# brown-palm/goal-force

Measured on AMD Instinct MI355X. Metric: frames_per_sec (81-frame video / (50-step denoise loop + VAE decode), Wan2.2-I2V-A14B 832x480x81f), higher is better.
Workload: dtype bf16

## Files before the change

goal_force_amd/csrc/gf_cross_fold.hip:

```cpp
#include "gf_common.h"

namespace {

constexpr int CF_HD = 128;
constexpr int CF_MAXK = 64;
constexpr int CF_THREADS = 256;
constexpr int CF_QB = 128;

__device__ __forceinline__ void cf_mfma32(f32x16& acc, const bf16x8& a, const bf16x8& b) {
    acc = __builtin_amdgcn_mfma_f32_32x32x16_bf16(a, b, acc, 0, 0, 0);
}

__global__ __launch_bounds__(CF_THREADS) void cross_probs_kernel(const u16* __restrict__ q, const u16* __restrict__ k, u16* __restrict__ pout,
                                                                 int q_len, int n_keys, int n_pad, int heads, long q_stride, long k_stride,
                                                                 long p_stride, float c, float last_key_bias) {
    __shared__ __attribute__((aligned(16))) char lds[CF_MAXK * 256];
    const int tid = threadIdx.x;
    const int lane = tid & 63, wave = tid >> 6;
    const int r = lane & 31, h = lane >> 5;
    const int head = blockIdx.y;
    const int q0 = blockIdx.x * CF_QB + wave * 32;
    const int halves = n_keys > 32 ? 2 : 1;

#pragma unroll
    for (int i = 0; i < (CF_MAXK * 16) / CF_THREADS; ++i) {
        const int idx = tid + CF_THREADS * i;
        const int row = idx >> 4, ch = idx & 15;
        u16x8 v8 = {0, 0, 0, 0, 0, 0, 0, 0};
        if (row < n_keys) v8 = *reinterpret_cast<const u16x8*>(k + (long)row * k_stride + head * CF_HD + ch * 8);
        const int sk = ((row & 3) << 2) | ((row >> 2) & 3);
        *(u16x8*)(lds + row * 256 + ((ch ^ sk) << 4)) = v8;
    }

    bf16x8 qf[8];
    {
        const int qr = min(q0 + r, q_len - 1);
        const u16* qp = q + (long)qr * q_stride + head * CF_HD + 8 * h;
#pragma unroll
        for (int kd = 0; kd < 8; ++kd) qf[kd] = *reinterpret_cast<const bf16x8*>(qp + 16 * kd);
    }
    __syncthreads();

    f32x16 sc[2];
#pragma unroll
    for (int e = 0; e < 16; ++e) {
        sc[0][e] = 0.f;
        sc[1][e] = 0.f;
    }
    const int sK = ((r & 3) << 2) | ((r >> 2) & 3);
#pragma unroll
    for (int kd = 0; kd < 8; ++kd) {
        const int off = 256 * r + 16 * ((2 * kd + h) ^ sK);
        cf_mfma32(sc[0], *(const bf16x8*)(lds + off), qf[kd]);
        if (halves == 2) cf_mfma32(sc[1], *(const bf16x8*)(lds + off + 32 * 256), qf[kd]);
    }

#pragma unroll
    for (int e = 0; e < 16; ++e) {
        const int key = 4 * h + (e & 3) + 8 * (e >> 2);
        if (key >= n_keys) sc[0][e] = -INFINITY;
        if (key + 32 >= n_keys) sc[1][e] = -INFINITY;
        if (key == n_keys - 1) sc[0][e] += last_key_bias;
        if (key + 32 == n_keys - 1) sc[1][e] += last_key_bias;
    }
    float mx = sc[0][0];
#pragma unroll
    for (int e = 1; e < 16; ++e) mx = fmaxf(mx, sc[0][e]);
#pragma unroll
    for (int e = 0; e < 16; ++e) mx = fmaxf(mx, sc[1][e]);
    mx = fmaxf(mx, __shfl_xor(mx, 32));
    const float mc = mx * c;
    float rs = 0.f;
#pragma unroll
    for (int e = 0; e < 16; ++e) {
        sc[0][e] = __builtin_amdgcn_exp2f(__builtin_fmaf(sc[0][e], c, -mc));
        sc[1][e] = __builtin_amdgcn_exp2f(__builtin_fmaf(sc[1][e], c, -mc));
        rs += sc[0][e] + sc[1][e];
    }
    const float l_tot = rs + __shfl_xor(rs, 32);
    const float inv = 1.0f / l_tot;
    float pl = 0.f;
#pragma unroll
    for (int e = 0; e < 16; ++e) {
        const int key = 4 * h + (e & 3) + 8 * (e >> 2);
        if (key == n_keys - 1) pl = sc[0][e];
        if (key + 32 == n_keys - 1) pl = sc[1][e];
    }
    pl += __shfl_xor(pl, 32);
    const float wl = pl * inv;
    const float wl_lo = wl - bf2f(f2bf(wl));

    const int qrow = q0 + r;
    if (qrow < q_len) {
        u16* prow = pout + (long)qrow * p_stride + (long)head * n_pad;
#pragma unroll
        for (int half = 0; half < 2; ++half)
#pragma unroll
            for (int g = 0; g < 4; ++g) {
                const int key = 32 * half + 8 * g + 4 * h;
                if (key < n_pad) {
                    float w4[4];
#pragma unroll
                    for (int i = 0; i < 4; ++i) w4[i] = key + i == n_keys ? wl_lo : sc[half][4 * g + i] * inv;
                    u32x2 pk;
                    pk[0] = pack2bf(w4[0], w4[1]);
                    pk[1] = pack2bf(w4[2], w4[3]);
                    *reinterpret_cast<u32x2*>(prow + key) = pk;
                }
            }
    }
}

constexpr int CFT_ROWS = 64;
__global__ __launch_bounds__(CF_THREADS) void cross_fold_table_kernel(const u16* __restrict__ v, const u16* __restrict__ w, u16* __restrict__ u,
                                                                      int n_keys, int n_pad, int n_out, long v_stride, long w_stride,
                                                                      long u_stride) {
    __shared__ __attribute__((aligned(16))) u16 vs[CF_MAXK * CF_HD];
    const int tid = threadIdx.x;
    const int head = blockIdx.y;
    for (int idx = tid; idx < n_pad * 16; idx += CF_THREADS) {
        const int row = idx >> 4, ch = idx & 15;
        u16x8 v8 = {0, 0, 0, 0, 0, 0, 0, 0};
        if (row <= n_keys) v8 = *reinterpret_cast<const u16x8*>(v + (long)min(row, n_keys - 1) * v_stride + head * CF_HD + ch * 8);
        *reinterpret_cast<u16x8*>(vs + row * CF_HD + ch * 8) = v8;
    }
    __syncthreads();
    const int n = blockIdx.x * CFT_ROWS + (tid >> 2), jg = tid & 3;
    if (n >= n_out) return;
    const int nj = n_pad >> 2;
    float acc[CF_MAXK / 4];
#pragma unroll
    for (int i = 0; i < CF_MAXK / 4; ++i) acc[i] = 0.f;
    const u16* wr = w + (long)n * w_stride + head * CF_HD;
    for (int d0 = 0; d0 < CF_HD; d0 += 8) {
        const u16x8 w8 = *reinterpret_cast<const u16x8*>(wr + d0);
        float wf[8];
#pragma unroll
        for (int e = 0; e < 8; ++e) wf[e] = bf2f(w8[e]);
#pragma unroll
        for (int i = 0; i < CF_MAXK / 4; ++i) {
            if (i < nj) {
                const u16x8 v8 = *reinterpret_cast<const u16x8*>(vs + (jg + 4 * i) * CF_HD + d0);
#pragma unroll
                for (int e = 0; e < 8; ++e) acc[i] = __builtin_fmaf(bf2f(v8[e]), wf[e], acc[i]);
            }
        }
    }
    u16* ur = u + (long)n * u_stride + (long)head * n_pad;
#pragma unroll
    for (int i = 0; i < CF_MAXK / 4; ++i) {
        const int j = jg + 4 * i;
        if (i < nj) ur[j] = j <= n_keys ? f2bf(acc[i]) : (u16)0;
    }
}

}

extern "C" GF_API int gf_cross_probs(const void* q, const void* k, void* p, int64_t q_len, int64_t n_keys, int64_t n_pad, int64_t heads,
                                     int64_t head_dim, int64_t q_stride, int64_t k_stride, int64_t p_stride, float scale,
                                     float last_key_multiplicity, void* stream) {
    GF_CHECK_ARG(q && k && p, "gf_cross_probs: null pointer");
    if (head_dim != CF_HD) {
        gf_set_error("gf_cross_probs: head_dim=%ld unsupported (kernel is built for 128)", (long)head_dim);
        return GF_ERR_UNSUPPORTED;
    }
    GF_CHECK_ARG(q_len >= 0 && q_len < (1 << 30) && heads > 0 && heads < 65536, "gf_cross_probs: bad sizes q=%ld heads=%ld", (long)q_len,
                 (long)heads);
    GF_CHECK_ARG(n_keys >= 1 && n_pad % 16 == 0 && n_pad > n_keys && n_pad <= CF_MAXK,
                 "gf_cross_probs: 1 <= n_keys=%ld < n_pad=%ld <= 64, n_pad a multiple of 16", (long)n_keys, (long)n_pad);
    GF_CHECK_ARG(q_stride % 8 == 0 && k_stride % 8 == 0 && p_stride % 4 == 0 && q_stride >= heads * CF_HD && k_stride >= heads * CF_HD &&
                     p_stride >= heads * n_pad,
                 "gf_cross_probs: strides must cover the rows (q, k: multiples of 8; p: of 4, >= heads * n_pad)");
    GF_CHECK_ARG(gf_aligned16(q) && gf_aligned16(k) && ((uintptr_t)p & 7u) == 0, "gf_cross_probs: alignment (q, k 16 bytes, p 8 bytes)");
    GF_CHECK_ARG(scale > 0.f && last_key_multiplicity >= 1.0f, "gf_cross_probs: scale > 0, multiplicity >= 1");
    if (q_len == 0) return GF_OK;
    const float c = scale * 1.4426950408889634f;
    const float bias = last_key_multiplicity != 1.0f ? log2f(last_key_multiplicity) / c : 0.f;
    const dim3 grid((unsigned)((q_len + CF_QB - 1) / CF_QB), (unsigned)heads);
    hipLaunchKernelGGL(cross_probs_kernel, grid, dim3(CF_THREADS), 0, (hipStream_t)stream, (const u16*)q, (const u16*)k, (u16*)p,
                       (int)q_len, (int)n_keys, (int)n_pad, (int)heads, (long)q_stride, (long)k_stride, (long)p_stride, c, bias);
    GF_CHECK_LAUNCH("gf_cross_probs");
    return GF_OK;
}

extern "C" GF_API int gf_cross_fold_table(const void* v, const void* w_o, void* u, int64_t n_keys, int64_t n_pad, int64_t heads,
                                          int64_t head_dim, int64_t n_out, int64_t v_stride, int64_t w_stride, int64_t u_stride,
                                          void* stream) {
    GF_CHECK_ARG(v && w_o && u, "gf_cross_fold_table: null pointer");
    if (head_dim != CF_HD) {
        gf_set_error("gf_cross_fold_table: head_dim=%ld unsupported (kernel is built for 128)", (long)head_dim);
        return GF_ERR_UNSUPPORTED;
    }
    GF_CHECK_ARG(heads > 0 && heads < 65536 && n_out > 0 && n_out < (1 << 30), "gf_cross_fold_table: bad sizes heads=%ld N=%ld", (long)heads,
                 (long)n_out);
    GF_CHECK_ARG(n_keys >= 1 && n_pad % 16 == 0 && n_pad > n_keys && n_pad <= CF_MAXK,
                 "gf_cross_fold_table: 1 <= n_keys=%ld < n_pad=%ld <= 64, n_pad a multiple of 16", (long)n_keys, (long)n_pad);
    GF_CHECK_ARG(v_stride % 8 == 0 && w_stride % 8 == 0 && v_stride >= heads * CF_HD && w_stride >= heads * CF_HD && u_stride >= heads * n_pad,
                 "gf_cross_fold_table: strides must cover the rows (v, w_o: multiples of 8; u >= heads * n_pad)");
    GF_CHECK_ARG(gf_aligned16(v) && gf_aligned16(w_o) && ((uintptr_t)u & 1u) == 0, "gf_cross_fold_table: alignment");
    const dim3 grid((unsigned)((n_out + CFT_ROWS - 1) / CFT_ROWS), (unsigned)heads);
    hipLaunchKernelGGL(cross_fold_table_kernel, grid, dim3(CF_THREADS), 0, (hipStream_t)stream, (const u16*)v, (const u16*)w_o, (u16*)u,
                       (int)n_keys, (int)n_pad, (int)n_out, (long)v_stride, (long)w_stride, (long)u_stride);
    GF_CHECK_LAUNCH("gf_cross_fold_table");
    return GF_OK;
}
```

goal_force_amd/dit.py:

```python
from __future__ import annotations

import math
from typing import Optional, Tuple

import torch
import torch.nn as nn

from . import ops
from ._lib import GoalForceError


def precompute_freqs_cis(dim: int, end: int = 1024, theta: float = 10000.0):
    freqs = 1.0 / (theta ** (torch.arange(0, dim, 2)[: (dim // 2)].double() / dim))
    freqs = torch.outer(torch.arange(end), freqs)
    return torch.polar(torch.ones_like(freqs), freqs)


def precompute_freqs_cis_3d(dim: int, end: int = 1024, theta: float = 10000.0):
    return (precompute_freqs_cis(dim - 2 * (dim // 3), end, theta),
            precompute_freqs_cis(dim // 3, end, theta),
            precompute_freqs_cis(dim // 3, end, theta))


class RopeTable:
# ... 283 lines not shown
        x2 = _tokens2d(x)
        a = self.attend(x2, _as_rope(freqs, x.device))
        return linear(a, self.o).view(x.shape)


class CrossAttention(nn.Module):

    def __init__(self, dim: int, num_heads: int, eps: float = 1e-6, has_image_input: bool = False):
        super().__init__()
        if has_image_input:
            raise NotImplementedError("has_image_input=True (CLIP image tokens) is outside the Goal-Force path")
        self.dim, self.num_heads, self.head_dim = dim, num_heads, dim // num_heads
        self.q, self.k, self.v, self.o = (nn.Linear(dim, dim) for _ in range(4))
        self.norm_q, self.norm_k = RMSNorm(dim, eps=eps), RMSNorm(dim, eps=eps)
        self.has_image_input = False

    def context_kv(self, ctx2: torch.Tensor, fold: bool = True, pad_n: Optional[int] = None):
        m = 1
        if fold and ctx2.is_cuda and ops._OPT["fold_pad_keys"]:
            n = pad_run(ctx2) if pad_n is None else pad_n
            if ctx2.shape[0] - n >= 2 and n + 1 < ops.VT_MIN_KV:
                m = ctx2.shape[0] - n
                ctx2 = ctx2[: n + 1]
        cin = QuantizedInput(ctx2) if getattr(self.k, "_gf_w8", None) is not None else ctx2
        k, v = linear(cin, self.k), linear(cin, self.v)
        ops.rmsnorm_rope(k, self.norm_k.weight, None, None, self.head_dim, self.norm_k.eps)
        return k, v, m

    def attend(self, x2, kv):
        q = linear(x2, self.q)
        ops.rmsnorm_rope(q, self.norm_q.weight, None, None, self.head_dim, self.norm_q.eps)
        return ops.flash_attn(q, kv[0], kv[1], self.num_heads, last_key_mult=kv[2] if len(kv) > 2 else 1)

    FOLD_K_MAX = 2560

    def fold_ok(self, kv) -> bool:
        if not ops._OPT["fold_cross_o"] or torch.is_grad_enabled() or len(kv) < 3 or kv[2] == 1 or self.head_dim != 128:
            return False
        if getattr(self.o, "_gf_w8", None) is not None:
            return False
        n = kv[0].shape[0]
        k = self.num_heads * self.fold_pad(n)
        return n <= ops.CROSS_FOLD_MAX_KEYS and k <= self.FOLD_K_MAX and k % 64 == 0

    @staticmethod
    def fold_pad(n_keys: int) -> int:
        return -(-(n_keys + 1) // 16) * 16

    def fold_table(self, kv):
        return ops.cross_fold_table(kv[1], self.o.weight, self.num_heads, self.fold_pad(kv[0].shape[0]))

    def attend_probs(self, x2, kv):
        q = linear(x2, self.q)
        ops.rmsnorm_rope(q, self.norm_q.weight, None, None, self.head_dim, self.norm_q.eps)
        return ops.cross_probs(q, kv[0], self.num_heads, self.fold_pad(kv[0].shape[0]), last_key_mult=kv[2])

    def forward(self, x: torch.Tensor, y: torch.Tensor):
        x2 = _tokens2d(x)
        a = self.attend(x2, self.context_kv(_tokens2d(y)))
        return linear(a, self.o).view(x.shape)


class GateModule(nn.Module):

    def forward(self, x, gate, residual):
        if x.shape != residual.shape:
            raise GoalForceError("GateModule: x and residual must have the same shape")
        d = x.shape[-1]
        g = gate.reshape(-1, d)
        if x.dim() == 3 and g.shape[0] == x.shape[0] and x.shape[0] > 1:
            return torch.stack([ops.gate_residual(x[b], g[b].contiguous(), residual[b]) for b in range(x.shape[0])])
        if g.shape[0] != 1:
            raise GoalForceError("GateModule: gate must be [B or 1, 1, D] (per-token gates are outside the Goal-Force path)")
        return ops.gate_residual(x, g[0].contiguous(), residual)


class DiTBlock(nn.Module):

    def __init__(self, has_image_input: bool, dim: int, num_heads: int, ffn_dim: int, eps: float = 1e-6):
        super().__init__()
        self.dim, self.num_heads, self.ffn_dim, self.eps = dim, num_heads, ffn_dim, eps
        self.self_attn = SelfAttention(dim, num_heads, eps)
        self.cross_attn = CrossAttention(dim, num_heads, eps, has_image_input=has_image_input)
        self.norm1 = nn.LayerNorm(dim, eps=eps, elementwise_affine=False)
        self.norm2 = nn.LayerNorm(dim, eps=eps, elementwise_affine=False)
        self.norm3 = nn.LayerNorm(dim, eps=eps)
        self.ffn = nn.Sequential(nn.Linear(dim, ffn_dim), nn.GELU(approximate="tanh"), nn.Linear(ffn_dim, dim))
        self.modulation = nn.Parameter(torch.randn(1, 6, dim) / dim ** 0.5)
        self.gate = GateModule()

    def forward(self, x, context, t_mod, freqs, context_kv=None, out=None, sp=None, keep=None, self_attn_memo=None,
                fold_pad_keys=True, pad_n=None, dense_attn=False):
        if t_mod.dim() == 4:
            raise NotImplementedError("per-token t_mod (seperated_timestep) is outside the Goal-Force path")
        x2 = _tokens2d(x)
        rope = _as_rope(freqs, x.device)
        mod = ops.modulation(self.modulation, t_mod.contiguous(), onep_mask=0b010010)
        fp8 = getattr(self.ffn[0], "_gf_w8", None) is not None
        if self_attn_memo is not None and "x" in self_attn_memo:
            x_new = self_attn_memo.pop("x")
            ev = self_attn_memo.pop("ev", None)
            if ev is not None:
                torch.cuda.current_stream(x_new.device).wait_event(ev)
                x_new.record_stream(torch.cuda.current_stream(x_new.device))
            if out is not None:
                x_new = out.copy_(x_new)
# ... 163 lines not shown
```

goal_force_amd/ops.py:

```python
from __future__ import annotations

import math

import torch

from . import _lib
from ._lib import (EPI_BIAS, EPI_BIAS_GATE_RESID, EPI_BIAS_GELU_TANH, EPI_BIAS_MUL, EPI_BIAS_RESID, EPI_BIAS_SILU,
                   GoalForceError)

__all__ = [
    "modulation", "layernorm_modulate", "rmsnorm_rope", "gate_residual", "gemm", "flash_attn", "flash_attn_sparse", "BlockMap", "patchify_im2col", "unpatchify",
    "cfg_euler_step", "act", "add", "sub", "rel_l1", "force_map",
    "EPI_BIAS", "EPI_BIAS_GELU_TANH", "EPI_BIAS_GATE_RESID", "EPI_BIAS_RESID", "EPI_BIAS_SILU", "EPI_BIAS_MUL",
]

_BF16 = torch.bfloat16
_FP8 = torch.float8_e4m3fn

PROFILE_ATTN = None
PROFILE_GEMM = None
PROFILE_CONV = None


def _stream(t: torch.Tensor):
# ... 169 lines not shown
        raise GoalForceError(f"gate_residual: residual must match x [{rows}, {dim}]")
    _vec(gate, "gate_residual.gate", dim, required=True)
    out = torch.empty(x.shape, dtype=_BF16, device=x.device)
    ov, _, _, os_ = _rows2d(out, "gate_residual.out")
    _lib.check(_lib.load().gf_gate_residual(_ptr(xv), _ptr(gate), _ptr(rv), _ptr(ov), rows, dim, xs, rs, os_, _stream(x)),
               "gf_gate_residual")
    return out


def rope_apply(x, cos, sin, head_dim):
    _req(x, "rope_apply.x")
    xv, rows, dim, xs = _rows2d(x, "rope_apply.x")
    for n, t in (("cos", cos), ("sin", sin)):
        _req(t, f"rope_apply.{n}", torch.float32)
        if tuple(t.shape) != (rows, head_dim // 2) or not t.is_contiguous():
            raise GoalForceError(f"rope_apply.{n}: expected contiguous [{rows}, {head_dim // 2}] fp32")
    out = torch.empty(x.shape, dtype=_BF16, device=x.device)
    ov, _, _, os_ = _rows2d(out, "rope_apply.out")
    _lib.check(_lib.load().gf_rope_apply(_ptr(xv), _ptr(ov), _ptr(cos), _ptr(sin), rows, dim, head_dim, xs, os_, _stream(x)),
               "gf_rope_apply")
    return out


def _gemm(a, w, row_scale, bias, epilogue, resid, gate, out):
    av, M, K, lda, N, ldw = _linear_operands(a, w, row_scale)
    if out is None:
        out = torch.empty(a.shape[:-1] + (N,), dtype=_BF16, device=a.device)
    ov, Mo, No, ldc = _rows2d(out, "gemm[_fp8].out")
    if (Mo, No) != (M, N):
        raise GoalForceError(f"gemm[_fp8].out: expected [{M}, {N}], got [{Mo}, {No}]")
    ldr = 0
    if resid is not None:
        _req(resid, "gemm[_fp8].resid")
        resid, Mr, Nr, ldr = _rows2d(resid, "gemm[_fp8].resid")
        if (Mr, Nr) != (M, N):
            raise GoalForceError(f"gemm[_fp8].resid: expected [{M}, {N}], got [{Mr}, {Nr}]")
    _vec(gate, "gemm[_fp8].gate", N)
    _vec(bias, "gemm[_fp8].bias", N)
    lib = _lib.load()
    fn, scale = (lib.gf_gemm_bf16, ()) if row_scale is None else (lib.gf_gemm_fp8, (_ptr(row_scale),))
    with _timed(PROFILE_GEMM, M, N, K, int(epilogue)):
        _lib.check(fn(_ptr(av), lda, _ptr(w), ldw, *scale, _ptr(bias), _ptr(ov), ldc, M, N, K, int(epilogue), _ptr(resid), ldr,
                      _ptr(gate), _stream(a)), fn.__name__)
    return out


def gemm(a, w, bias=None, epilogue=EPI_BIAS, resid=None, gate=None, out=None):
    return _gemm(a, w, None, bias, epilogue, resid, gate, out)


VT_MIN_KV = 2048
_LIB_DEFAULTS = {"prefer_8wave": 0, "a4_stagger": 2, "a4_group_m": 0, "conv_nb": 0, "conv_gather": 0, "conv_direct": 1, "vae_rms3": 1}
_OPT = {"attn_k3": True, "vt_from_gemm": True, "conv_padded": True, "fold_pad_keys": True, "attn_q_prescale": True, "vae_attn_offset": True,
        "fold_cross_o": True}


def lib_option(name: str) -> int:
    import ctypes
    v = ctypes.c_int(0)
    _lib.check(_lib.load().gf_get_option(name.encode(), ctypes.byref(v)), f"gf_get_option({name})")
    return int(v.value)


class options:

    def __init__(self, **kv):
        for k in kv:
            if k not in _OPT and k not in _LIB_DEFAULTS:
                raise GoalForceError(f"ops.options: unknown option {k!r}")
        self.kv, self.old = kv, {}

    @staticmethod
    def _apply_one(k, v):
        if k in _OPT:
            _OPT[k] = bool(v)
        else:
            _lib.check(_lib.load().gf_set_option(k.encode(), int(v)), f"gf_set_option({k})")

    def __enter__(self):
        self.old = {}
        try:
            for k, v in self.kv.items():
                old = _OPT[k] if k in _OPT else lib_option(k)
                self._apply_one(k, v)
                self.old[k] = old
        except BaseException:
            self.__exit__(None, None, None)
            raise
        return self

    def __exit__(self, *exc):
        for k, v in reversed(list(self.old.items())):
            self._apply_one(k, v)
        self.old = {}
        return False


_VT_WS = {}


def _vt_workspace(numel, device):
    key = (device.index, torch.cuda.current_stream(device).cuda_stream)
    ws = _VT_WS.get(key)
    if ws is None or ws.numel() < numel:
        ws = _VT_WS[key] = torch.empty((numel,), dtype=_BF16, device=device)
    return ws

# ... 245 lines not shown
        skv, ldv, src, vt_in = kv_len, kv_pad(kv_len), vt, 1
        if vt.numel() < num_heads * 128 * ldv:
            raise GoalForceError("sage_quant_vt.vt: buffer smaller than heads*128*kv_pad")
    kv_pad8 = -(-skv // SAGE_T) * SAGE_T
    vt8 = torch.empty((num_heads * 128, kv_pad8), dtype=torch.uint8, device=src.device)
    sc = torch.empty((num_heads, 128), dtype=torch.float32, device=src.device)
    _lib.check(_lib.load().gf_sage_quant_vt(_ptr(src), ldv, vt_in, _ptr(vt8), _ptr(sc), _ptr(_sage_scratch(num_heads, src.device)), skv,
                                            num_heads, _stream(src)), "gf_sage_quant_vt")
    return vt8, sc


def sage_attn_quantized(q8, q_scale, k8, k_scale, vt8, v_scale, kv_len, num_heads, scale=None, out=None):
    sq = q8.shape[0]
    scale = _sage_scale(scale)
    if out is None:
        out = torch.empty((sq, num_heads * 128), dtype=_BF16, device=q8.device)
    _lib.check(_lib.load().gf_sage_attn_fwd(_ptr(q8), _ptr(q_scale), _ptr(k8), _ptr(k_scale), _ptr(vt8), _ptr(v_scale), _ptr(out),
                                            out.stride(0), sq, kv_len, num_heads, scale, _stream(q8)), "gf_sage_attn_fwd")
    return out


def sage_attn(q, k, v, num_heads, scale=None, vt=None, out=None):
    scale = _sage_scale(scale)
    sq, ldq = _sage_rows(q, "sage_attn.q", num_heads)
    skv, ldk = _sage_rows(k, "sage_attn.k", num_heads)
    if vt is None:
        sv, ldv = _sage_rows(v, "sage_attn.v", num_heads)
        if sv != skv:
            raise GoalForceError(f"sage_attn: k has {skv} keys, v {sv}")
        src, vt_in = v, 0
    else:
        _req(vt, "sage_attn.vt")
        ldv, src, vt_in = kv_pad(skv), vt, 1
        if vt.numel() < num_heads * 128 * ldv:
            raise GoalForceError("sage_attn.vt: buffer smaller than heads*128*kv_pad")
    out = _out(out, "sage_attn.out", sq, num_heads * 128, q.device)
    if out.stride(0) % 8:
        raise GoalForceError("sage_attn.out: row stride must be a multiple of 8 elements")
    lib = _lib.load()
    nbytes = int(lib.gf_sage_workspace_bytes(sq, skv, num_heads))
    key = (q.device.index, torch.cuda.current_stream(q.device).cuda_stream)
    ws = _SAGE_WS.get(key)
    if ws is None or ws.numel() < nbytes:
        ws = _SAGE_WS[key] = torch.empty((nbytes,), dtype=torch.uint8, device=q.device)
    with _timed(PROFILE_ATTN, sq, skv, num_heads):
        _lib.check(lib.gf_sage_attn(_ptr(q), ldq, _ptr(k), ldk, _ptr(src), ldv, vt_in, _ptr(out), out.stride(0), sq, skv, num_heads,
                                    scale, _ptr(ws), _stream(q)), "gf_sage_attn")
    return out


CROSS_FOLD_MAX_KEYS = 63


def cross_probs(q, k, num_heads, n_pad, last_key_mult=1, scale=None, out=None):
    _mat(q, "cross_probs.q")
    _mat(k, "cross_probs.k")
    sq, hd_all = q.shape
    n_keys = k.shape[0]
    head_dim = hd_all // num_heads
    if k.shape[1] != hd_all or head_dim * num_heads != hd_all:
        raise GoalForceError("cross_probs: q/k shape mismatch")
    out = _out(out, "cross_probs.out", sq, num_heads * n_pad, q.device)
    if scale is None:
        scale = 1.0 / math.sqrt(head_dim)
    _lib.check(_lib.load().gf_cross_probs(_ptr(q), _ptr(k), _ptr(out), sq, n_keys, n_pad, num_heads, head_dim, q.stride(0), k.stride(0),
                                          out.stride(0), float(scale), float(last_key_mult), _stream(q)), "gf_cross_probs")
    return out


def cross_fold_table(v, w_o, num_heads, n_pad):
    _mat(v, "cross_fold_table.v")
    n_keys, hd_all = v.shape
    N, ldw = _weight(w_o, "cross_fold_table.w_o", hd_all)
    if hd_all % num_heads:
        raise GoalForceError(f"cross_fold_table: {hd_all} columns do not divide into {num_heads} heads")
    u = torch.empty((N, num_heads * n_pad), dtype=_BF16, device=v.device)
    _lib.check(_lib.load().gf_cross_fold_table(_ptr(v), _ptr(w_o), _ptr(u), n_keys, n_pad, num_heads, hd_all // num_heads, N, v.stride(0),
                                               ldw, u.stride(0), _stream(v)), "gf_cross_fold_table")
    return u


def flash_attn_lse(q, k, v, num_heads, scale=None):
    for n, t in (("q", q), ("k", k), ("v", v)):
        _mat(t, f"flash_attn_lse.{n}")
    sq, hd_all = q.shape
    skv = k.shape[0]
    head_dim = hd_all // num_heads
    if k.shape[1] != hd_all or v.shape != k.shape or head_dim * num_heads != hd_all:
        raise GoalForceError("flash_attn_lse: q/k/v shape mismatch")
    if scale is None:
        scale = 1.0 / math.sqrt(head_dim)
    out = torch.empty((sq, hd_all), dtype=_BF16, device=q.device)
    lse = torch.empty((sq, num_heads), dtype=torch.float32, device=q.device)
    lib = _lib.load()
    if _vt_shape(skv, num_heads, head_dim):
        _vt_attn(lib, q, k, v, None, out, lse, sq, skv, num_heads, head_dim, scale, _OPT["attn_k3"])
        return out, lse
    _lib.check(lib.gf_flash_attn_fwd_lse(_ptr(q), _ptr(k), _ptr(v), _ptr(out), _ptr(lse), sq, skv, num_heads, head_dim,
                                         q.stride(0), k.stride(0), v.stride(0), out.stride(0), float(scale),
                                         _stream(q)), "gf_flash_attn_fwd_lse")
    return out, lse


def flash_attn_bwd(q, k, v, o, dout, lse, num_heads, scale=None, need_dkv=True):
    for n, t in (("q", q), ("k", k), ("v", v), ("o", o), ("dout", dout)):
        _mat(t, f"flash_attn_bwd.{n}")
    sq, hd_all = q.shape
    skv = k.shape[0]
    head_dim = hd_all // num_heads
    if scale is None:
        scale = 1.0 / math.sqrt(head_dim)
    if lse.dtype != torch.float32 or tuple(lse.shape) != (sq, num_heads) or not lse.is_contiguous():
        raise GoalForceError("flash_attn_bwd.lse: expected contiguous fp32 [Sq, heads]")
    dq = torch.empty_like(q, memory_format=torch.contiguous_format)
    dk = torch.empty((skv, hd_all), dtype=_BF16, device=q.device) if need_dkv else None
    dv = torch.empty((skv, hd_all), dtype=_BF16, device=q.device) if need_dkv else None
    lib = _lib.load()
# ... 480 lines not shown
```

include/goalforce.h:

```cpp
#ifndef GOALFORCE_H
#define GOALFORCE_H

#include <stdint.h>

#if defined(GF_BUILD)
#define GF_API __attribute__((visibility("default")))
#else
#define GF_API
#endif

#ifdef __cplusplus
extern "C" {
#endif

typedef enum {
    GF_OK = 0,
    GF_ERR_INVALID_ARG = -1,
    GF_ERR_UNSUPPORTED = -2,
    GF_ERR_LAUNCH = -3
} gf_status;

GF_API const char* gf_version(void);
GF_API const char* gf_last_error(void);
#define GF_ABI_VERSION 20
// ... 11 lines not shown
                         int64_t t_rows, uint32_t onep_mask, void* stream);

GF_API int gf_rmsnorm_rope(void* x, const void* weight, const float* cos_tab, const float* sin_tab,
                    int64_t rows, int64_t dim, int64_t head_dim, int64_t x_stride,
                    float eps, void* stream);

typedef enum {
    GF_EPI_BIAS = 0,
    GF_EPI_BIAS_GELU_TANH = 1,
    GF_EPI_BIAS_GATE_RESID = 2,
    GF_EPI_BIAS_RESID = 3,
    GF_EPI_BIAS_SILU = 4,
    GF_EPI_BIAS_MUL = 5
} gf_epilogue;

GF_API int gf_gemm_bf16(const void* A, int64_t lda, const void* W, int64_t ldw, const void* bias,
                 void* C, int64_t ldc, int64_t M, int64_t N, int64_t K,
                 int epilogue, const void* resid, int64_t ldr, const void* gate,
                 void* stream);

GF_API int gf_gemm_bf16_batched(const void* A, int64_t lda, int64_t strideA, const void* W, int64_t ldw, int64_t strideW, void* C,
                                int64_t ldc, int64_t strideC, int64_t M, int64_t N, int64_t K, int64_t batch, void* stream);

GF_API int gf_flash_attn_fwd(const void* q, const void* k, const void* v, void* o,
                      int64_t q_len, int64_t kv_len, int64_t heads, int64_t head_dim,
                      int64_t q_stride, int64_t k_stride, int64_t v_stride, int64_t o_stride,
                      float scale, void* stream);

GF_API int gf_transpose_v(const void* v, int64_t v_stride, void* vt, int64_t kv_len, int64_t kv_pad, int64_t heads, void* stream);
GF_API int gf_flash_attn_fwd_vt(const void* q, const void* k, const void* vt, void* o, float* lse,
                         int64_t q_len, int64_t kv_len, int64_t kv_pad, int64_t heads, int64_t head_dim,
                         int64_t q_stride, int64_t k_stride, int64_t o_stride, float scale, void* stream);

GF_API int gf_transpose_v32(const void* v, int64_t v_stride, void* vt, int64_t kv_len, int64_t kv_pad, int64_t heads, void* stream);
GF_API int gf_flash_attn_fwd_vt32(const void* q, const void* k, const void* vt, void* o, float* lse,
                                  int64_t q_len, int64_t kv_len, int64_t kv_pad, int64_t heads, int64_t head_dim,
                                  int64_t q_stride, int64_t k_stride, int64_t o_stride, float scale, void* stream);

GF_API int gf_flash_attn_fwd_vt32_sparse(const void* q, const void* k, const void* vt, void* o, float* lse,
                                         const int32_t* row_ptr, const int32_t* tile_idx, const int32_t* head_map, int64_t n_maps,
                                         int64_t q_len, int64_t kv_len, int64_t kv_pad, int64_t heads, int64_t head_dim,
                                         int64_t q_stride, int64_t k_stride, int64_t o_stride, float scale, void* stream);

GF_API int gf_linear_vt32(const void* x, int64_t ldx, const void* w, int64_t ldw, const void* bias, void* vt,
                          int64_t kv_len, int64_t kv_pad, int64_t N, int64_t K, void* stream);

GF_API int gf_flash_attn_fwd_lastmult(const void* q, const void* k, const void* v, void* o, int64_t q_len, int64_t kv_len,
                                      int64_t heads, int64_t head_dim, int64_t q_stride, int64_t k_stride, int64_t v_stride,
                                      int64_t o_stride, float scale, float last_key_multiplicity, void* stream);

GF_API int gf_cross_probs(const void* q, const void* k, void* p, int64_t q_len, int64_t n_keys, int64_t n_pad, int64_t heads,
                          int64_t head_dim, int64_t q_stride, int64_t k_stride, int64_t p_stride, float scale,
                          float last_key_multiplicity, void* stream);

GF_API int gf_cross_fold_table(const void* v, const void* w_o, void* u, int64_t n_keys, int64_t n_pad, int64_t heads, int64_t head_dim,
                               int64_t n_out, int64_t v_stride, int64_t w_stride, int64_t u_stride, void* stream);

GF_API int gf_flash_attn_fwd_lse(const void* q, const void* k, const void* v, void* o, float* lse,
                          int64_t q_len, int64_t kv_len, int64_t heads, int64_t head_dim,
                          int64_t q_stride, int64_t k_stride, int64_t v_stride, int64_t o_stride,
                          float scale, void* stream);
GF_API int64_t gf_flash_attn_bwd_workspace_bytes(int64_t q_len, int64_t kv_len, int64_t heads);
GF_API int gf_flash_attn_bwd(const void* q, const void* k, const void* v, const void* o, const void* dout,
                      const float* lse, void* workspace, void* dq, void* dk, void* dv,
                      int64_t q_len, int64_t kv_len, int64_t heads, int64_t head_dim,
                      int64_t q_stride, int64_t k_stride, int64_t v_stride, int64_t o_stride, int64_t do_stride,
                      int64_t dq_stride, int64_t dk_stride, int64_t dv_stride, float scale, void* stream);

GF_API int gf_layernorm_bwd(const void* x, int64_t x_stride, const void* dy, int64_t dy_stride, const void* g, void* dx,
                            int64_t dx_stride, float* dg_acc, float* db_acc, int64_t rows, int64_t dim, float eps, void* stream);
GF_API int gf_rmsnorm_rope_bwd(const void* x, int64_t x_stride, const void* dy, int64_t dy_stride, const void* weight,
                               const float* cos_tab, const float* sin_tab, void* dx, int64_t dx_stride, float* dw_acc,
                               int64_t rows, int64_t dim, int64_t head_dim, float eps, void* stream);
GF_API int gf_colsum(const void* a, int64_t lda, const void* b, int64_t ldb, const void* gate, void* out, int64_t ldo,
                     float* acc, int64_t rows, int64_t cols, void* stream);
GF_API int gf_act_bwd(const void* u, const void* df, void* du, int64_t n, int kind, void* stream);
GF_API int gf_mse_loss(const void* pred, const void* target, void* dpred, float* loss, int64_t n, float weight, void* stream);
GF_API int gf_adamw_step(void* param, const void* grad, float* exp_avg, float* exp_avg_sq, int64_t n, float lr, float beta1,
                         float beta2, float eps, float weight_decay, int64_t step, float grad_scale, void* stream);
GF_API int gf_f32_to_bf16(const float* src, void* dst, int64_t n, void* stream);
GF_API int gf_sumsq(const void* x, int64_t n, float* acc, void* stream);

GF_API int gf_patchify_im2col(const void* src0, int64_t c0, const void* src1, int64_t c1,
                       void* out, int64_t F, int64_t H, int64_t W, int64_t kpad, void* stream);

GF_API int gf_unpatchify(const void* tokens, void* out, int64_t c, int64_t f, int64_t h, int64_t w,
                  void* stream);

GF_API int gf_cfg_euler_step(void* latents, const void* posi, const void* nega,
                      float cfg_scale, float dsigma, int64_t n, void* stream);

GF_API int gf_act(const void* x, void* out, int64_t n, int kind, void* stream);

GF_API int gf_add_bf16(const void* a, const void* b, void* out, int64_t n, void* stream);

GF_API int gf_sub_bf16(const void* a, const void* b, void* out, int64_t n, void* stream);
GF_API int gf_rel_l1_bf16(const void* cur, const void* prev, int64_t n, void* sums, void* stream);

GF_API int gf_force_map(void* out, int64_t frames, int64_t H, int64_t W,
                 const int32_t* channels, const float* params, const float* centers,
                 int64_t n_blobs, int clamp01, void* stream);


GF_API int gf_vae_prep_latent(const void* z, int64_t sc, int64_t st, int64_t sy, int64_t sx,
                              const void* mean, const void* inv_std, void* out,
                              int64_t C, int64_t T, int64_t H, int64_t W, int64_t cpad, void* stream);
// ... 92 lines not shown
```

Measured before the change: 0.6211.

## Fuse query RMSNorm into cross-attention probability kernel

Adds a cross_probs_norm kernel that computes the per-row RMS statistic of the query across all heads and applies the norm weight on the fly while computing cross-attention probabilities. Each block now loops over a range of heads, double-buffering key tiles in shared memory and prefetching the next head's queries and keys. This removes the separate rmsnorm pass that read and rewrote the full query tensor. In exchange the grid shrinks to one block per query tile with a serial head loop, so parallelism and occupancy are lower, and it only supports 40 or 4 heads.

```diff
diff --git a/goal_force_amd/csrc/gf_cross_fold.hip b/goal_force_amd/csrc/gf_cross_fold.hip
--- a/goal_force_amd/csrc/gf_cross_fold.hip
+++ b/goal_force_amd/csrc/gf_cross_fold.hip
@@ -1,4 +1,5 @@
 #include "gf_common.h"
+#include "gf_rms_row.h"
 
 namespace {
 
@@ -9,6 +10,89 @@
 
 __device__ __forceinline__ void cf_mfma32(f32x16& acc, const bf16x8& a, const bf16x8& b) {
     acc = __builtin_amdgcn_mfma_f32_32x32x16_bf16(a, b, acc, 0, 0, 0);
+}
+
+__device__ __forceinline__ u16x8 cf_key_chunk(const u16* __restrict__ k, int idx, int head, int n_keys, long k_stride) {
+    const int row = idx >> 4, ch = idx & 15;
+    u16x8 v8 = {0, 0, 0, 0, 0, 0, 0, 0};
+    if (row < n_keys) v8 = *reinterpret_cast<const u16x8*>(k + (long)row * k_stride + head * CF_HD + ch * 8);
+    return v8;
+}
+__device__ __forceinline__ void cf_key_store(char* lds, int idx, u16x8 v8) {
+    const int row = idx >> 4, ch = idx & 15;
+    const int sk = ((row & 3) << 2) | ((row >> 2) & 3);
+    *(u16x8*)(lds + row * 256 + ((ch ^ sk) << 4)) = v8;
+}
+
+__device__ __forceinline__ void cf_head_probs(const char* lds, const bf16x8 (&qf)[8], u16* prow, int r, int h, int n_keys, int n_pad, float c,
+                                              float last_key_bias) {
+    const int halves = n_keys > 32 ? 2 : 1;
+    f32x16 sc[2];
+#pragma unroll
+    for (int e = 0; e < 16; ++e) {
+        sc[0][e] = 0.f;
+        sc[1][e] = 0.f;
+    }
+    const int sK = ((r & 3) << 2) | ((r >> 2) & 3);
+#pragma unroll
+    for (int kd = 0; kd < 8; ++kd) {
+        const int off = 256 * r + 16 * ((2 * kd + h) ^ sK);
+        cf_mfma32(sc[0], *(const bf16x8*)(lds + off), qf[kd]);
+        if (halves == 2) cf_mfma32(sc[1], *(const bf16x8*)(lds + off + 32 * 256), qf[kd]);
+    }
+
+#pragma unroll
+    for (int e = 0; e < 16; ++e) {
+        const int key = 4 * h + (e & 3) + 8 * (e >> 2);
+        if (key >= n_keys) sc[0][e] = -INFINITY;
+        if (key + 32 >= n_keys) sc[1][e] = -INFINITY;
+        if (key == n_keys - 1) sc[0][e] += last_key_bias;
+        if (key + 32 == n_keys - 1) sc[1][e] += last_key_bias;
+    }
+    float mx = sc[0][0];
+#pragma unroll
+    for (int e = 1; e < 16; ++e) mx = fmaxf(mx, sc[0][e]);
+#pragma unroll
+    for (int e = 0; e < 16; ++e) mx = fmaxf(mx, sc[1][e]);
+    mx = fmaxf(mx, __shfl_xor(mx, 32));
+    const float mc = mx * c;
+    float rs = 0.f;
+#pragma unroll
+    for (int e = 0; e < 16; ++e) {
+        sc[0][e] = __builtin_amdgcn_exp2f(__builtin_fmaf(sc[0][e], c, -mc));
+        sc[1][e] = __builtin_amdgcn_exp2f(__builtin_fmaf(sc[1][e], c, -mc));
+        rs += sc[0][e] + sc[1][e];
+    }
+    const float l_tot = rs + __shfl_xor(rs, 32);
+    const float inv = 1.0f / l_tot;
+    float pl = 0.f;
+#pragma unroll
+    for (int e = 0; e < 16; ++e) {
+        const int key = 4 * h + (e & 3) + 8 * (e >> 2);
+        if (key == n_keys - 1) pl = sc[0][e];
+        if (key + 32 == n_keys - 1) pl = sc[1][e];
+    }
+    pl += __shfl_xor(pl, 32);
+    const float wl = pl * inv;
+    const float wl_lo = wl - bf2f(f2bf(wl));
+
+    if (prow) {
+#pragma unroll
+        for (int half = 0; half < 2; ++half)
+#pragma unroll
+            for (int g = 0; g < 4; ++g) {
+                const int key = 32 * half + 8 * g + 4 * h;
+                if (key < n_pad) {
+                    float w4[4];
+#pragma unroll
+                    for (int i = 0; i < 4; ++i) w4[i] = key + i == n_keys ? wl_lo : sc[half][4 * g + i] * inv;
+                    u32x2 pk;
+                    pk[0] = pack2bf(w4[0], w4[1]);
+                    pk[1] = pack2bf(w4[2], w4[3]);
+                    *reinterpret_cast<u32x2*>(prow + key) = pk;
+                }
+            }
+    }
 }
 
 __global__ __launch_bounds__(CF_THREADS) void cross_probs_kernel(const u16* __restrict__ q, const u16* __restrict__ k, u16* __restrict__ pout,
@@ -20,16 +104,11 @@
     const int r = lane & 31, h = lane >> 5;
     const int head = blockIdx.y;
     const int q0 = blockIdx.x * CF_QB + wave * 32;
-    const int halves = n_keys > 32 ? 2 : 1;
 
 #pragma unroll
     for (int i = 0; i < (CF_MAXK * 16) / CF_THREADS; ++i) {
         const int idx = tid + CF_THREADS * i;
-        const int row = idx >> 4, ch = idx & 15;
-        u16x8 v8 = {0, 0, 0, 0, 0, 0, 0, 0};
-        if (row < n_keys) v8 = *reinterpret_cast<const u16x8*>(k + (long)row * k_stride + head * CF_HD + ch * 8);
-        const int sk = ((row & 3) << 2) | ((row >> 2) & 3);
-        *(u16x8*)(lds + row * 256 + ((ch ^ sk) << 4)) = v8;
+        cf_key_store(lds, idx, cf_key_chunk(k, idx, head, n_keys, k_stride));
     }
 
     bf16x8 qf[8];
@@ -40,74 +119,86 @@
         for (int kd = 0; kd < 8; ++kd) qf[kd] = *reinterpret_cast<const bf16x8*>(qp + 16 * kd);
     }
     __syncthreads();
-
-    f32x16 sc[2];
-#pragma unroll
-    for (int e = 0; e < 16; ++e) {
-        sc[0][e] = 0.f;
-        sc[1][e] = 0.f;
-    }
-    const int sK = ((r & 3) << 2) | ((r >> 2) & 3);
+    const int qrow = q0 + r;
+    cf_head_probs(lds, qf, qrow < q_len ? pout + (long)qrow * p_stride + (long)head * n_pad : nullptr, r, h, n_keys, n_pad, c, last_key_bias);
+}
+
+constexpr int CFN_U = 4;
+constexpr int CFN_SETS = 2;
+constexpr int CFN_THREADS = CF_THREADS * CFN_SETS;
+template <int NCH>
+__global__ __launch_bounds__(CFN_THREADS) void cross_probs_norm_kernel(const u16* __restrict__ q, const u16* __restrict__ k,
+                                                                       const u16* __restrict__ g, u16* __restrict__ pout, int q_len,
+                                                                       int n_keys, int n_pad, long q_stride, long k_stride, long p_stride,
+                                                                       float c, float last_key_bias, float eps) {
+    constexpr int HPS = NCH * 4 / CFN_SETS;
+    constexpr int KCH = (CF_MAXK * 16) / CF_THREADS;
+    __shared__ __attribute__((aligned(16))) char lds[CFN_SETS][2][CF_MAXK * 256];
+    const int tid = threadIdx.x;
+    const int lane = tid & 63, wave = (tid >> 6) & 3, set = tid >> 8, tset = tid & (CF_THREADS - 1);
+    const int r = lane & 31, h = lane >> 5;
+    const int qb = blockIdx.x * CF_QB;
+    const int q0 = qb + wave * 32;
+    const int head0 = set * HPS;
+
+    u16x8 kreg[KCH];
+#pragma unroll
+    for (int i = 0; i < KCH; ++i) kreg[i] = cf_key_chunk(k, tset + CF_THREADS * i, head0, n_keys, k_stride);
+
+    float* rstd_s = reinterpret_cast<float*>(lds[0][1]);
+    for (int i0 = 0; i0 < 16; i0 += CFN_U) {
+        u16x8 v[CFN_U][NCH];
+        float rs[CFN_U];
+        const int row0 = wave * 32 + set * 16 + i0;
+#pragma unroll
+        for (int u = 0; u < CFN_U; ++u) rs[u] = rms_row_rstd<NCH>(q + (long)min(qb + row0 + u, q_len - 1) * q_stride + lane * 8, v[u], eps);
+#pragma unroll
+        for (int u = 0; u < CFN_U; ++u)
+            if (lane == 0) rstd_s[row0 + u] = rs[u];
+    }
+
+    const int qr = min(q0 + r, q_len - 1);
+    const u16* qp = q + (long)qr * q_stride + head0 * CF_HD + 8 * h;
+    const u16* gp = g + head0 * CF_HD + 8 * h;
+    u16x8 qn[8], gn[8];
 #pragma unroll
     for (int kd = 0; kd < 8; ++kd) {
-        const int off = 256 * r + 16 * ((2 * kd + h) ^ sK);
-        cf_mfma32(sc[0], *(const bf16x8*)(lds + off), qf[kd]);
-        if (halves == 2) cf_mfma32(sc[1], *(const bf16x8*)(lds + off + 32 * 256), qf[kd]);
-    }
-
-#pragma unroll
-    for (int e = 0; e < 16; ++e) {
-        const int key = 4 * h + (e & 3) + 8 * (e >> 2);
-        if (key >= n_keys) sc[0][e] = -INFINITY;
-        if (key + 32 >= n_keys) sc[1][e] = -INFINITY;
-        if (key == n_keys - 1) sc[0][e] += last_key_bias;
-        if (key + 32 == n_keys - 1) sc[1][e] += last_key_bias;
-    }
-    float mx = sc[0][0];
-#pragma unroll
-    for (int e = 1; e < 16; ++e) mx = fmaxf(mx, sc[0][e]);
-#pragma unroll
-    for (int e = 0; e < 16; ++e) mx = fmaxf(mx, sc[1][e]);
-    mx = fmaxf(mx, __shfl_xor(mx, 32));
-    const float mc = mx * c;
-    float rs = 0.f;
-#pragma unroll
-    for (int e = 0; e < 16; ++e) {
-        sc[0][e] = __builtin_amdgcn_exp2f(__builtin_fmaf(sc[0][e], c, -mc));
-        sc[1][e] = __builtin_amdgcn_exp2f(__builtin_fmaf(sc[1][e], c, -mc));
-        rs += sc[0][e] + sc[1][e];
-    }
-    const float l_tot = rs + __shfl_xor(rs, 32);
-    const float inv = 1.0f / l_tot;
-    float pl = 0.f;
-#pragma unroll
-    for (int e = 0; e < 16; ++e) {
-        const int key = 4 * h + (e & 3) + 8 * (e >> 2);
-        if (key == n_keys - 1) pl = sc[0][e];
-        if (key + 32 == n_keys - 1) pl = sc[1][e];
-    }
-    pl += __shfl_xor(pl, 32);
-    const float wl = pl * inv;
-    const float wl_lo = wl - bf2f(f2bf(wl));
+        qn[kd] = *reinterpret_cast<const u16x8*>(qp + 16 * kd);
+        gn[kd] = *reinterpret_cast<const u16x8*>(gp + 16 * kd);
+    }
+#pragma unroll
+    for (int i = 0; i < KCH; ++i) cf_key_store(lds[set][0], tset + CF_THREADS * i, kreg[i]);
+    __syncthreads();
+    const float rstd = rstd_s[wave * 32 + r];
+    __syncthreads();
 
     const int qrow = q0 + r;
-    if (qrow < q_len) {
-        u16* prow = pout + (long)qrow * p_stride + (long)head * n_pad;
-#pragma unroll
-        for (int half = 0; half < 2; ++half)
-#pragma unroll
-            for (int g = 0; g < 4; ++g) {
-                const int key = 32 * half + 8 * g + 4 * h;
-                if (key < n_pad) {
-                    float w4[4];
-#pragma unroll
-                    for (int i = 0; i < 4; ++i) w4[i] = key + i == n_keys ? wl_lo : sc[half][4 * g + i] * inv;
-                    u32x2 pk;
-                    pk[0] = pack2bf(w4[0], w4[1]);
-                    pk[1] = pack2bf(w4[2], w4[3]);
-                    *reinterpret_cast<u32x2*>(prow + key) = pk;
-                }
+    u16* prow = qrow < q_len ? pout + (long)qrow * p_stride + (long)head0 * n_pad : nullptr;
+    for (int hh = 0; hh < HPS; ++hh) {
+        bf16x8 qf[8];
+#pragma unroll
+        for (int kd = 0; kd < 8; ++kd) {
+            u16x8 o;
+#pragma unroll
+            for (int j = 0; j < 8; ++j) o[j] = f2bf(rms_row_scale(qn[kd][j], rstd, gn[kd][j]));
+            qf[kd] = __builtin_bit_cast(bf16x8, o);
+        }
+        const bool more = hh + 1 < HPS;
+        if (more) {
+#pragma unroll
+            for (int i = 0; i < KCH; ++i) kreg[i] = cf_key_chunk(k, tset + CF_THREADS * i, head0 + hh + 1, n_keys, k_stride);
+#pragma unroll
+            for (int kd = 0; kd < 8; ++kd) {
+                qn[kd] = *reinterpret_cast<const u16x8*>(qp + (hh + 1) * CF_HD + 16 * kd);
+                gn[kd] = *reinterpret_cast<const u16x8*>(gp + (hh + 1) * CF_HD + 16 * kd);
             }
+        }
+        cf_head_probs(lds[set][hh & 1], qf, prow ? prow + (long)hh * n_pad : nullptr, r, h, n_keys, n_pad, c, last_key_bias);
+        if (more) {
+#pragma unroll
+            for (int i = 0; i < KCH; ++i) cf_key_store(lds[set][(hh + 1) & 1], tset + CF_THREADS * i, kreg[i]);
+        }
+        __syncthreads();
     }
 }
 
@@ -156,30 +247,65 @@
 
 }
 
+static int cross_probs_check(const char* fn, const void* q, const void* k, void* p, int64_t q_len, int64_t n_keys, int64_t n_pad, int64_t heads,
+                             int64_t head_dim, int64_t q_stride, int64_t k_stride, int64_t p_stride, float scale, float last_key_multiplicity,
+                             float* c, float* bias) {
+    GF_CHECK_ARG(q && k && p, "%s: null pointer", fn);
+    if (head_dim != CF_HD) {
+        gf_set_error("%s: head_dim=%ld unsupported (kernel is built for 128)", fn, (long)head_dim);
+        return GF_ERR_UNSUPPORTED;
+    }
+    GF_CHECK_ARG(q_len >= 0 && q_len < (1 << 30) && heads > 0 && heads < 65536, "%s: bad sizes q=%ld heads=%ld", fn, (long)q_len, (long)heads);
+    GF_CHECK_ARG(n_keys >= 1 && n_pad % 16 == 0 && n_pad > n_keys && n_pad <= CF_MAXK, "%s: 1 <= n_keys=%ld < n_pad=%ld <= 64, n_pad a multiple of 16", fn,
+                 (long)n_keys, (long)n_pad);
+    GF_CHECK_ARG(q_stride % 8 == 0 && k_stride % 8 == 0 && p_stride % 4 == 0 && q_stride >= heads * CF_HD && k_stride >= heads * CF_HD &&
+                     p_stride >= heads * n_pad,
+                 "%s: strides must cover the rows (q, k: multiples of 8; p: of 4, >= heads * n_pad)", fn);
+    GF_CHECK_ARG(gf_aligned16(q) && gf_aligned16(k) && ((uintptr_t)p & 7u) == 0, "%s: alignment (q, k 16 bytes, p 8 bytes)", fn);
+    GF_CHECK_ARG(scale > 0.f && last_key_multiplicity >= 1.0f, "%s: scale > 0, multiplicity >= 1", fn);
+    *c = scale * 1.4426950408889634f;
+    *bias = last_key_multiplicity != 1.0f ? log2f(last_key_multiplicity) / *c : 0.f;
+    return GF_OK;
+}
+
 extern "C" GF_API int gf_cross_probs(const void* q, const void* k, void* p, int64_t q_len, int64_t n_keys, int64_t n_pad, int64_t heads,
                                      int64_t head_dim, int64_t q_stride, int64_t k_stride, int64_t p_stride, float scale,
                                      float last_key_multiplicity, void* stream) {
-    GF_CHECK_ARG(q && k && p, "gf_cross_probs: null pointer");
-    if (head_dim != CF_HD) {
-        gf_set_error("gf_cross_probs: head_dim=%ld unsupported (kernel is built for 128)", (long)head_dim);
-        return GF_ERR_UNSUPPORTED;
-    }
-    GF_CHECK_ARG(q_len >= 0 && q_len < (1 << 30) && heads > 0 && heads < 65536, "gf_cross_probs: bad sizes q=%ld heads=%ld", (long)q_len,
-                 (long)heads);
-    GF_CHECK_ARG(n_keys >= 1 && n_pad % 16 == 0 && n_pad > n_keys && n_pad <= CF_MAXK,
-                 "gf_cross_probs: 1 <= n_keys=%ld < n_pad=%ld <= 64, n_pad a multiple of 16", (long)n_keys, (long)n_pad);
-    GF_CHECK_ARG(q_stride % 8 == 0 && k_stride % 8 == 0 && p_stride % 4 == 0 && q_stride >= heads * CF_HD && k_stride >= heads * CF_HD &&
-                     p_stride >= heads * n_pad,
-                 "gf_cross_probs: strides must cover the rows (q, k: multiples of 8; p: of 4, >= heads * n_pad)");
-    GF_CHECK_ARG(gf_aligned16(q) && gf_aligned16(k) && ((uintptr_t)p & 7u) == 0, "gf_cross_probs: alignment (q, k 16 bytes, p 8 bytes)");
-    GF_CHECK_ARG(scale > 0.f && last_key_multiplicity >= 1.0f, "gf_cross_probs: scale > 0, multiplicity >= 1");
+    float c, bias;
+    const int rc = cross_probs_check("gf_cross_probs", q, k, p, q_len, n_keys, n_pad, heads, head_dim, q_stride, k_stride, p_stride, scale,
+                                     last_key_multiplicity, &c, &bias);
+    if (rc != GF_OK) return rc;
     if (q_len == 0) return GF_OK;
-    const float c = scale * 1.4426950408889634f;
-    const float bias = last_key_multiplicity != 1.0f ? log2f(last_key_multiplicity) / c : 0.f;
     const dim3 grid((unsigned)((q_len + CF_QB - 1) / CF_QB), (unsigned)heads);
     hipLaunchKernelGGL(cross_probs_kernel, grid, dim3(CF_THREADS), 0, (hipStream_t)stream, (const u16*)q, (const u16*)k, (u16*)p,
                        (int)q_len, (int)n_keys, (int)n_pad, (int)heads, (long)q_stride, (long)k_stride, (long)p_stride, c, bias);
     GF_CHECK_LAUNCH("gf_cross_probs");
+    return GF_OK;
+}
+
+extern "C" GF_API int gf_cross_probs_norm(const void* q, const void* norm_weight, const void* k, void* p, int64_t q_len, int64_t n_keys,
+                                          int64_t n_pad, int64_t heads, int64_t head_dim, int64_t q_stride, int64_t k_stride, int64_t p_stride,
+                                          float scale, float last_key_multiplicity, float eps, void* stream) {
+    float c, bias;
+    const int rc = cross_probs_check("gf_cross_probs_norm", q, k, p, q_len, n_keys, n_pad, heads, head_dim, q_stride, k_stride, p_stride, scale,
+                                     last_key_multiplicity, &c, &bias);
+    if (rc != GF_OK) return rc;
+    GF_CHECK_ARG(norm_weight && gf_aligned16(norm_weight), "gf_cross_probs_norm: norm_weight (16-byte aligned) required");
+    if (heads != 40 && heads != 4) {
+        gf_set_error("gf_cross_probs_norm: heads=%ld unsupported (40 or 4: the widths whose gf_rmsnorm_rope sum is reproduced, gf_rms_row.h)", (long)heads);
+        return GF_ERR_UNSUPPORTED;
+    }
+    if (q_len == 0) return GF_OK;
+    const dim3 grid((unsigned)((q_len + CF_QB - 1) / CF_QB));
+    if (heads == 40)
+        hipLaunchKernelGGL(cross_probs_norm_kernel<10>, grid, dim3(CFN_THREADS), 0, (hipStream_t)stream, (const u16*)q, (const u16*)k,
+                           (const u16*)norm_weight, (u16*)p, (int)q_len, (int)n_keys, (int)n_pad, (long)q_stride, (long)k_stride, (long)p_stride, c,
+                           bias, eps);
+    else
+        hipLaunchKernelGGL(cross_probs_norm_kernel<1>, grid, dim3(CFN_THREADS), 0, (hipStream_t)stream, (const u16*)q, (const u16*)k,
+                           (const u16*)norm_weight, (u16*)p, (int)q_len, (int)n_keys, (int)n_pad, (long)q_stride, (long)k_stride, (long)p_stride, c,
+                           bias, eps);
+    GF_CHECK_LAUNCH("gf_cross_probs_norm");
     return GF_OK;
 }
 
diff --git a/goal_force_amd/csrc/gf_rms_row.h b/goal_force_amd/csrc/gf_rms_row.h
--- /dev/null
+++ b/goal_force_amd/csrc/gf_rms_row.h
@@ -0,0 +1,25 @@
+#pragma once
+#include "gf_common.h"
+
+template <int NCH>
+__device__ __forceinline__ float rms_row_rstd(const u16* xr, u16x8 (&v)[NCH], float eps) {
+#pragma clang fp contract(off)
+    constexpr int DIM = NCH * 512;
+    float s = 0.f;
+#pragma unroll
+    for (int i = 0; i < NCH; ++i) {
+        v[i] = *reinterpret_cast<const u16x8*>(xr + i * 512);
+#pragma unroll
+        for (int j = 0; j < 8; ++j) {
+            const float f = bf2f(v[i][j]);
+            const float f2 = f * f;
+            s = s + f2;
+        }
+    }
+    return 1.0f / sqrtf(__builtin_fmaf(wave_sum(s), 1.0f / DIM, eps));
+}
+
+__device__ __forceinline__ float rms_row_scale(u16 x, float rstd, u16 w) {
+    const float n = rbf(bf2f(x) * rstd);
+    return rbf(n * bf2f(w));
+}
diff --git a/goal_force_amd/dit.py b/goal_force_amd/dit.py
--- a/goal_force_amd/dit.py
+++ b/goal_force_amd/dit.py
@@ -359,6 +359,9 @@
 
     def attend_probs(self, x2, kv):
         q = linear(x2, self.q)
+        if ops.cross_norm_ok(self.num_heads, self.head_dim):
+            return ops.cross_probs(q, kv[0], self.num_heads, self.fold_pad(kv[0].shape[0]), last_key_mult=kv[2],
+                                   norm_weight=self.norm_q.weight, eps=self.norm_q.eps)
         ops.rmsnorm_rope(q, self.norm_q.weight, None, None, self.head_dim, self.norm_q.eps)
         return ops.cross_probs(q, kv[0], self.num_heads, self.fold_pad(kv[0].shape[0]), last_key_mult=kv[2])
 
diff --git a/goal_force_amd/ops.py b/goal_force_amd/ops.py
--- a/goal_force_amd/ops.py
+++ b/goal_force_amd/ops.py
@@ -245,7 +245,7 @@
 VT_MIN_KV = 2048
 _LIB_DEFAULTS = {"prefer_8wave": 0, "a4_stagger": 2, "a4_group_m": 0, "conv_nb": 0, "conv_gather": 0, "conv_direct": 1, "vae_rms3": 1}
 _OPT = {"attn_k3": True, "vt_from_gemm": True, "conv_padded": True, "fold_pad_keys": True, "attn_q_prescale": True, "vae_attn_offset": True,
-        "fold_cross_o": True}
+        "fold_cross_o": True, "cross_probs_norm": True}
 
 
 def lib_option(name: str) -> int:
@@ -597,7 +597,14 @@
 CROSS_FOLD_MAX_KEYS = 63
 
 
-def cross_probs(q, k, num_heads, n_pad, last_key_mult=1, scale=None, out=None):
+CROSS_NORM_HEADS = (40, 4)
+
+
+def cross_norm_ok(num_heads, head_dim):
+    return _OPT["cross_probs_norm"] and head_dim == 128 and num_heads in CROSS_NORM_HEADS
+
+
+def cross_probs(q, k, num_heads, n_pad, last_key_mult=1, scale=None, out=None, norm_weight=None, eps=1e-6):
     _mat(q, "cross_probs.q")
     _mat(k, "cross_probs.k")
     sq, hd_all = q.shape
@@ -608,6 +615,12 @@
     out = _out(out, "cross_probs.out", sq, num_heads * n_pad, q.device)
     if scale is None:
         scale = 1.0 / math.sqrt(head_dim)
+    if norm_weight is not None:
+        _vec(norm_weight, "cross_probs.norm_weight", hd_all)
+        _lib.check(_lib.load().gf_cross_probs_norm(_ptr(q), _ptr(norm_weight), _ptr(k), _ptr(out), sq, n_keys, n_pad, num_heads, head_dim,
+                                                   q.stride(0), k.stride(0), out.stride(0), float(scale), float(last_key_mult), float(eps),
+                                                   _stream(q)), "gf_cross_probs_norm")
+        return out
     _lib.check(_lib.load().gf_cross_probs(_ptr(q), _ptr(k), _ptr(out), sq, n_keys, n_pad, num_heads, head_dim, q.stride(0), k.stride(0),
                                           out.stride(0), float(scale), float(last_key_mult), _stream(q)), "gf_cross_probs")
     return out
diff --git a/include/goalforce.h b/include/goalforce.h
--- a/include/goalforce.h
+++ b/include/goalforce.h
@@ -87,6 +87,10 @@
 GF_API int gf_cross_probs(const void* q, const void* k, void* p, int64_t q_len, int64_t n_keys, int64_t n_pad, int64_t heads,
                           int64_t head_dim, int64_t q_stride, int64_t k_stride, int64_t p_stride, float scale,
                           float last_key_multiplicity, void* stream);
+
+GF_API int gf_cross_probs_norm(const void* q, const void* norm_weight, const void* k, void* p, int64_t q_len, int64_t n_keys,
+                               int64_t n_pad, int64_t heads, int64_t head_dim, int64_t q_stride, int64_t k_stride, int64_t p_stride,
+                               float scale, float last_key_multiplicity, float eps, void* stream);
 
 GF_API int gf_cross_fold_table(const void* v, const void* w_o, void* u, int64_t n_keys, int64_t n_pad, int64_t heads, int64_t head_dim,
                                int64_t n_out, int64_t v_stride, int64_t w_stride, int64_t u_stride, void* stream);
```

Result: no change. 0.6222 (median of 6 runs) (+0.2%).
